# HK-SHAO/RayTracingPBR

Hardware: AMD Instinct MI355X
Metric: Msamples/sec (pixels x spp / s), Cornell Box 1920x1080 (higher is better)
Workload: dtype f32

## Files before the change

### raytracingpbr_amd/csrc/rt_capi.hip

```cpp
#include <hip/hip_runtime.h>

#include <cmath>
#include <cstdio>
#include <cstdlib>
#include <cstring>
#include <string>
#include <vector>

#include "rt_ctx.hpp"
#include "rt_features.hpp"
#include "rt_reproject.hpp"
#include "rt_noise.hpp"
#include "rt_present.hpp"
#include "rt_select.hpp"

using namespace rt;

static void derive_launch(rtpbr_ctx* c, RtJitKey* key, bool* want, bool* strict_error);
static int noise_alloc(rtpbr_ctx* c);
extern "C" int rtpbr_set_option(rtpbr_ctx* c, const char* key, long long value);
extern "C" int rtpbr_set_tiles(rtpbr_ctx* c, int tw, int th, int rank, int world);
extern "C" int rtpbr_set_camera(rtpbr_ctx* c, const rtpbr_camera* cam);

static thread_local char g_err[512];
// ... 648 lines not shown
        if (((mask >> b) & 1u) && c->read_pending[b] >= 0) {
            const hipError_t q = hipEventQuery(c->ev_read_done[c->read_pending[b] & 7]);
            if (q == hipErrorNotReady) {
                (void)hipGetLastError();
                HIP_TRY(hipStreamWaitEvent(c->stream, c->ev_read_done[c->read_pending[b] & 7], 0));
            } else if (q != hipSuccess) {
                return rt_fail_hip("hipEventQuery(read-back)", q);
            }
            c->read_pending[b] = -1;
        }
    return RTPBR_OK;
}
enum : unsigned { W_IMAGE_BUFFER = 1u << RTPBR_BUF_IMAGE_BUFFER, W_IMAGE_PIXELS = 1u << RTPBR_BUF_IMAGE_PIXELS, W_RAY_BUFFER = 1u << RTPBR_BUF_RAY_BUFFER,
                W_DIFF_BUFFER = 1u << RTPBR_BUF_DIFF_BUFFER, W_DIFF_PIXELS = 1u << RTPBR_BUF_DIFF_PIXELS };

extern "C" int rtpbr_refresh(rtpbr_ctx* c) {
    if (!c || !c->have_cfg) return fail(RTPBR_ESTATE, "set_config first");
    if (int r = set_dev(c)) return r;
    if (int r = flush_shade(c)) return r;
    if (int r = rt_order_after_reads(c, W_IMAGE_BUFFER | W_RAY_BUFFER | W_DIFF_BUFFER | W_DIFF_PIXELS | (c->noise_moments ? 1u << RTPBR_BUF_MOMENTS : 0u))) return r;
    size_t n = (size_t)c->cfg.width * c->cfg.height;
    if (c->noise_moments) {
        HIP_TRY(hipMemsetAsync(c->noise_moments, 0, n * sizeof(float4), c->stream));
        HIP_TRY(hipMemsetAsync(c->noise_snapshot, 0, n * sizeof(float4), c->stream));
    }
    launch_refresh(c->image_buffer, c->ray_buffer, c->diff_buffer, c->diff_pixels, c->cfg.adaptive_sampling, n, c->stream);
    HIP_TRY(hipGetLastError());
    c->history_ok = true;
    return RTPBR_OK;
}

static void pack_objects(rtpbr_ctx* c, Params& P) { pack_table(c->objm, c->n_obj, P.box_sig, P.objm); }

constexpr size_t PRIMARY_REC_BYTES = 5;
constexpr size_t STAGE_ITEM_BYTES = 14;
constexpr uint32_t DENSE_CHUNK_MIN = 32, DENSE_CHUNK_MAX = 256, DENSE_BATCH_MAX = 4096;
static size_t stage_bytes(size_t items) { return items * sizeof(StageRec) + (items / DENSE_CHUNK_MIN + 2) * sizeof(uint32_t) + items; }
static int staging_alloc(rtpbr_ctx* c, void** ptr, size_t* cap, size_t need) {
    if (need <= *cap) return RTPBR_OK;
    HIP_TRY(hipStreamSynchronize(c->stream));
    (void)hipFree(*ptr);
    *ptr = nullptr;
    *cap = 0;
    const hipError_t e = hipMalloc(ptr, need);
    if (e == hipErrorOutOfMemory) {
        (void)hipGetLastError();
        *ptr = nullptr;
        return RTPBR_ENOMEM;
    }
    if (e != hipSuccess) return rt_fail_hip("hipMalloc(staging)", e);
    *cap = need;
    return RTPBR_OK;
}
static int ensure_staging(rtpbr_ctx* c, size_t items, bool split, bool stage = true) {
    if (stage)
        if (int r = staging_alloc(c, (void**)&c->stage, &c->stage_cap, stage_bytes(items))) return r;
    if (split)
        if (int r = staging_alloc(c, (void**)&c->primary, &c->primary_cap, items * PRIMARY_REC_BYTES)) return r;
    return RTPBR_OK;
}

static int next_event_of(std::vector<hipEvent_t>& pool, int& used, hipEvent_t* out) {
    if (used == (int)pool.size()) {
        hipEvent_t e = nullptr;
        HIP_TRY(hipEventCreateWithFlags(&e, hipEventDisableSystemFence));
        pool.push_back(e);
    }
// ... 312 lines not shown
            c->shade_pending_base = P.sample_base;
            c->shade_pending_same_call = true;
        }
    }
    P.sparse_lanes = sparse_saved;
    return rc;
}

static int sample_complete_path(rtpbr_ctx* c, int n, bool selected = false) {
    Params& P = c->P;
    int left = n;
    if (int r = flush_shade(c)) return r;
    c->dense_launches = 0;
    const bool tracked = c->noise_tracking == RTPBR_NOISE_TRACK_SAMPLES;
    while (left > 0) {
        const bool split_ok = !selected && c->primary_split && P.scheduler == 1 && c->kind != KIND_BUNNY && c->kind != KIND_MIXED;
        const bool unstaged = c->precision != 0 && c->jit_mod != nullptr && P.scheduler == 1;
        long long per_spp = (long long)P.np * (long long)((unstaged ? 0 : STAGE_ITEM_BYTES) + (split_ok ? PRIMARY_REC_BYTES : 0));
        if (per_spp < 1) per_spp = 1;
        long long kmax = c->staging_bytes / per_spp;
        if (kmax < 1) kmax = 1;
        long long k32 = (0xFFFFFFFFLL - work_margin(c)) / (long long)P.np;
        if (k32 < 1) k32 = 1;
        if (kmax > k32) kmax = k32;
        int K = (int)(left < kmax ? left : kmax);
        const bool split = split_ok && (c->primary_split == 2 || (long long)P.np * K >= tune::PRIMARY_SPLIT_MIN_ITEMS);
        if (int r = ensure_staging(c, (size_t)P.np * (size_t)K, split, !unstaged)) {
            if (r != RTPBR_ENOMEM || K == 1)
                return r == RTPBR_ENOMEM ? fail(RTPBR_ENOMEM, "no device memory for the staging of one sample per pixel") : r;
            c->staging_bytes = (long long)((K + 1) / 2) * per_spp;
            continue;
        }
        P.primary = c->primary;
        P.primary_code = reinterpret_cast<uint8_t*>(c->primary + (size_t)P.np * (size_t)K);
        P.primary_split = split ? 1 : 0;
        P.primary_lean = c->primary_lean;
        P.drain_lanes = c->drain_lanes;
        P.stage = c->stage;
        P.K = K;
        P.sample_base = c->sample_base;
        P.total_items = (uint32_t)((long long)P.np * K);
        int grid = trace_grid(c, P.total_items, selected);
        long long waves = (long long)grid * tune::WAVES_PER_BLOCK;
        long long chunk = (long long)P.total_items / (waves * 64);
        if (chunk < tune::CHUNK_MIN) chunk = (long long)P.total_items < waves * tune::CHUNK_MIN ? tune::CHUNK_TINY : tune::CHUNK_MIN;
        if (chunk > tune::CHUNK_MAX) chunk = tune::CHUNK_MAX;
        if (c->chunk > 0) chunk = c->chunk;
        P.chunk = (uint32_t)chunk;
        P.stage_dense = 0;
        if (c->stage_dense && c->jit_mod != nullptr && !unstaged && P.scheduler == 1 && !tracked) {
            long long lo = DENSE_CHUNK_MIN, hi = chunk < 64 ? 64 : chunk > (long long)DENSE_CHUNK_MAX ? (long long)DENSE_CHUNK_MAX : chunk, cc = 0;
            if (c->chunk > 0) lo = hi = c->chunk;
            if (lo >= (long long)DENSE_CHUNK_MIN && hi <= (long long)DENSE_CHUNK_MAX)
                for (long long t = hi; t >= lo; t--)
                    if (t % K == 0 || K % t == 0) { cc = t; break; }
            const long long unit = cc > K ? cc : K;
            if (cc > 0 && unit <= (long long)DENSE_BATCH_MAX) {
                P.chunk = (uint32_t)cc;
                P.stage_dense = 1;
                c->dense_launches++;
                P.acc_batch = (uint32_t)(unit * ((long long)DENSE_BATCH_MAX / unit));
                P.acc_magic_k = K > 1 ? (uint32_t)(0x100000000ULL / (unsigned long long)K) + 1u : 0u;
                P.acc_magic_chunk = (uint32_t)(0x100000000ULL / (unsigned long long)cc) + 1u;
                const size_t n_fill = (size_t)P.total_items / (size_t)cc + 1;
                P.stage_fill = reinterpret_cast<uint32_t*>(c->stage + (size_t)P.total_items * 3u);
                P.stage_idx = reinterpret_cast<uint8_t*>(P.stage_fill + n_fill);
                HIP_TRY(hipMemsetAsync(P.stage_fill, 0, n_fill * sizeof(uint32_t), c->stream));
            }
// ... 1021 lines not shown
    } else if (!strcmp(key, "tiny_own")) {
        if (value < 0 || value > 128) return fail(RTPBR_EINVAL, "tiny_own must be 0 (no small heavy waves) .. 128");
        c->tiny_own = (int)value;
    } else if (!strcmp(key, "leave_x8")) {
        if (value < 1 || value > 4096) return fail(RTPBR_EINVAL, "leave_x8 must be 1 .. 4096 (eighths of a march iteration)");
        c->leave_x8 = (int)value;
    } else if (!strcmp(key, "heavy_prio")) {
        if (value < 0 || value > 1) return fail(RTPBR_EINVAL, "heavy_prio must be 0 or 1");
        c->heavy_prio = (int)value;
    } else if (!strcmp(key, "heavy_mean_x16")) {
        if (value < 0 || value > (1 << 20)) return fail(RTPBR_EINVAL, "heavy_mean_x16 must be 0 .. 2^20");
        c->heavy_mean_x16 = (int)value;
    } else if (!strcmp(key, "heavy_bulk_x16")) {
        if (value < 0 || value > (1 << 20)) return fail(RTPBR_EINVAL, "heavy_bulk_x16 must be 0 .. 2^20");
        c->heavy_bulk_x16 = (int)value;
    } else if (!strcmp(key, "grid_blocks")) {
        if (value < 0 || value > 65535) return fail(RTPBR_EINVAL, "grid_blocks must be 0 (automatic) .. 65535");
        c->grid_blocks = (int)value;
    } else if (!strcmp(key, "residency")) {
        if (value < 1 || value > 256 || (value & (value - 1))) return fail(RTPBR_EINVAL, "residency must be a power of two, 1..256");
        c->residency = (int)value;
    } else if (!strcmp(key, "ready_low")) {
        if (value < 0 || value > 63) return fail(RTPBR_EINVAL, "ready_low must be 0..63");
        c->ready_low = (int)value;
    } else if (!strcmp(key, "refill_lanes")) {
        if (value < 1 || value > 64) return fail(RTPBR_EINVAL, "refill_lanes must be 1..64");
        c->refill_lanes = (int)value;
    } else if (!strcmp(key, "timing")) {
        if (value < 0 || value > 1) return fail(RTPBR_EINVAL, "timing must be 0 or 1");
        c->timing = (int)value;
    } else if (!strcmp(key, "stage_dense")) {
        if (value < 0 || value > 1) return fail(RTPBR_EINVAL, "stage_dense must be 0 (item-linear staging) or 1 (records appended per claim in completion order)");
        c->stage_dense = (int)value;
    } else if (!strcmp(key, "primary_split")) {
        if (value < 0 || value > 2) return fail(RTPBR_EINVAL, "primary_split must be 0 (never), 1 (large launches) or 2 (always)");
        c->primary_split = (int)value;
    } else if (!strcmp(key, "drain_lanes")) {
        if (value < 0 || value > 64) return fail(RTPBR_EINVAL, "drain_lanes must be 0..64");
        c->drain_lanes = (int)value;
    } else if (!strcmp(key, "primary_lean")) {
        if (value < 0 || value > 1) return fail(RTPBR_EINVAL, "primary_lean must be 0 or 1");
        c->primary_lean = (int)value;
    } else if (!strcmp(key, "lazy_sqrt")) {
        if (value < 0 || value > 1) return fail(RTPBR_EINVAL, "lazy_sqrt must be 0 or 1");
        c->lazy_sqrt = (int)value;
    } else if (!strcmp(key, "jit")) {
        if (value < -1 || value > 2)
            return fail(RTPBR_EINVAL, "jit must be -1 (when no ahead-of-time specialisation fits), 0 (never), 1 (always, falling back to the "
                                      "ahead-of-time instance if compilation is impossible) or 2 (always, an error otherwise)");
        c->jit = (int)value;
    } else if (!strcmp(key, "precision")) {
        if (value < 0 || value > 1) return fail(RTPBR_EINVAL, "precision must be 0 (exactly rounded, the default) or 1 (tolerance flavour: hardware sqrt / rcp / sin / exp, contraction)");
        c->precision = (int)value;
    } else if (!strcmp(key, "jit_bake")) {
        if (value < 0 || value > 2) return fail(RTPBR_EINVAL, "jit_bake must be 0, 1 (scene + configuration) or 2 (+ the camera frame: fixed-camera offline renders)");
        c->jit_bake = (int)value;
    } else if (!strcmp(key, "specialize")) {
        if (value < 0 || value > 1) return fail(RTPBR_EINVAL, "specialize must be 0 or 1");
        c->specialize = (int)value;
    } else if (!strcmp(key, "mlp_mfma")) {
        if (value < 0 || value > 1) return fail(RTPBR_EINVAL, "mlp_mfma must be 0 or 1");
        c->mlp_mfma = (int)value;
    } else if (!strcmp(key, "mlp_lanes")) {
        if (value < 1 || value > 64) return fail(RTPBR_EINVAL, "mlp_lanes must be 1..64");
        c->mlp_lanes = (int)value;
    } else if (!strcmp(key, "mlp_full")) {
// ... 72 lines not shown
```

### raytracingpbr_amd/csrc/rt_ctx.hpp

```cpp
#pragma once
#include <hip/hip_runtime.h>

#include <string>
#include <vector>

#include "rt_device.hpp"
#include "rt_noise.hpp"
#include "rt_present.hpp"
#include "rt_select.hpp"

namespace rt {
void launch_trace(const Params& P, int kind, int grid, hipStream_t st);
void launch_accumulate(const Params& P, int n_cu, hipStream_t st);
void launch_trace_selected(const Params& P, int kind, int grid, hipStream_t st);
void launch_accumulate_selected(const Params& P, hipStream_t st);
void launch_accumulate_tracked(const Params& P, float4* moments, float4* snapshot, hipStream_t st);
void launch_accumulate_selected_tracked(const Params& P, float4* moments, float4* snapshot, hipStream_t st);
int trace_selected_blocks_per_cu(int kind, int n_obj, int scheduler);
void launch_zero(void* p, size_t bytes, hipStream_t st);
void launch_persistent(const Params& P, int kind, int steps, hipStream_t st);
void launch_persistent_pool(const Params& P, int kind, int steps, int grid, hipStream_t st);
int persistent_pool_blocks_per_cu(int kind);
void launch_chain_steps(const Params& P, int kind, int steps, int grid, hipStream_t st);
void launch_src_gen(const Params& P, int kind, hipStream_t st);
// ... 60 lines not shown
    using Params = rt::Params;
    using ObjFull = rt::ObjFull;
    using ObjM = rt::ObjM;
    using Counters = rt::Counters;
    static constexpr int MAX_OBJ = rt::MAX_OBJ;
    int device = 0;
    bool headless = false;
    hipStream_t stream = nullptr;
    bool have_cfg = false, have_scene = false, have_cam = false;
    rtpbr_config cfg{};
    rtpbr_object obj[MAX_OBJ];
    int n_obj = 0;
    int kind = rt::KIND_GENERIC;
    rtpbr_camera cam{};
    Params P{};
    float4* image_buffer = nullptr;
    float* image_pixels = nullptr;
    rtpbr_ray* ray_buffer = nullptr;
    float2* diff_buffer = nullptr;
    float* diff_pixels = nullptr;
    ObjFull* objfull = nullptr;
    float4* env = nullptr;
    uint32_t* env8 = nullptr;
    float* env_lut = nullptr;
    int env_packed = 1;
    float* bunny = nullptr;
    float* stage = nullptr;
    size_t stage_cap = 0;
    float* primary = nullptr;
    size_t primary_cap = 0;
    int drain_lanes = 16;
    int primary_lean = 1;
    int primary_split = 1;
    int specialize = 1;
    int lazy_sqrt = 1;
    uint32_t scene_sig = 0;
    ObjM objm[MAX_OBJ];
    unsigned int* work_counter = nullptr;
    int timing = 1;
    bool total1_recorded = false;
    Counters* counters = nullptr;
    Counters* counters_buf[2] = {nullptr, nullptr};
    bool counters_clean[2] = {false, false};
    int counters_turn = 0;
    int tile_w = 0, tile_h = 0, rank = 0, world = 1;
    uint32_t sample_base = 0;
    long long staging_bytes = 16LL << 30;
    int wait_lanes = 24;
    int shade_lanes = 56;
    int refill_lanes = 24;
    int ready_low = 4;
    int jit_waves = 0;
    int chunk = 0;
    int stage_dense = 0;
    unsigned long long dense_launches = 0;
    int residency = 32;
    int sparse_lanes = 24;
    int src_plan = 1;
    int plan_interval = 64;
    int heavy_own = 80;
    int age_on = 1;
    int age_w[8] = {8, 8, 8, 8, 8, 8, 8, 8};
    int tiny_waves = 64;
    int tiny_own = 8;
    int leave_x8 = 24;
    int src_track = 2;
    int src_op = 7;
    int heavy_prio = 1;
    int heavy_mean_x16 = 48;
    int heavy_bulk_x16 = 8;
    uint32_t* cost_buffer = nullptr;
    unsigned int* team_counter = nullptr;
    std::vector<void*> host_blocks;
    std::vector<size_t> host_sizes;
    hipStream_t copy_stream = nullptr;
    hipEvent_t ev_read_ready = nullptr;
    hipEvent_t ev_read_done[8] = {};
    int read_issued = 0;
    int read_pending[15] = {-1, -1, -1, -1, -1, -1, -1, -1, -1, -1, -1, -1, -1, -1, -1};
    uint32_t* march_out = nullptr;
// ... 84 lines not shown
```

### raytracingpbr_amd/csrc/rt_trace.hpp

```cpp
#pragma once
#include <hip/hip_runtime.h>

#include "rt_device.hpp"

namespace rt {

RT_D uint32_t wave_sum(uint32_t v) {
#pragma unroll
    for (int off = 32; off > 0; off >>= 1) v += __shfl_xor(v, off, 64);
    return v;
}

RT_D void flush_counters(const Params& P, uint32_t steps, uint32_t raycasts, uint32_t hits, uint32_t sky,
                         uint32_t samples, uint32_t deposits) {
    __shared__ unsigned long long blk[6];
    if (threadIdx.x < 6) blk[threadIdx.x] = 0;
    __syncthreads();
    steps = wave_sum(steps);
    raycasts = wave_sum(raycasts);
    hits = wave_sum(hits);
    sky = wave_sum(sky);
    samples = wave_sum(samples);
    deposits = wave_sum(deposits);
    if ((threadIdx.x & 63) == 0) {
// ... 140 lines not shown
}
RT_D void acc_flush_all(const Params& P, const AccView& A, int lane, uint32_t& n_dep) {
    lds_wave_fence();
    for (uint32_t s = 0; s < (uint32_t)ACC_SLOTS; s++) {
        const uint32_t t = (uint32_t)__builtin_amdgcn_readfirstlane((int)A.tag[s]);
        if (t != 0xffffffffu) acc_flush_slot(P, A, s, t, lane, n_dep);
    }
}

template <bool LIST = false>
RT_D int start_item(const Params& P, PathRay& R) {
    uint32_t q = R.item / (uint32_t)P.K;
    uint32_t k = R.item - q * (uint32_t)P.K;
    int px, py;
    if constexpr (LIST) {
        const uint32_t i = P.order[q];
        px = (int)(i / (uint32_t)P.cfg.height);
        py = (int)(i - (uint32_t)px * (uint32_t)P.cfg.height);
    } else {
        if (!pixel_of(P, q, px, py)) return -1;
    }
    R.key = rng_key(P.cfg.seed, (uint32_t)px, (uint32_t)py, P.sample_base + k);
    R.cnt = 0;
    gen_ray(P, px, py, R.key, R.cnt, R.o, R.d);
    R.col = mk(1, 1, 1);
    R.bounce = 0;
    float inv_pdf = exp_(0.0f / P.cfg.light_quality);
    float p = 1.0f - 1.0f / inv_pdf;
    if (rng_next(R.key, R.cnt) < p) {
        R.col = R.col * p;
        return 0;
    }
    return 1;
}

struct WorkRange {
    uint32_t next, end;
    bool drained;
};

RT_D bool claim_items(const Params& P, WorkRange& wr, bool want, int lane, uint32_t& item) {
    const unsigned long long m = __ballot(want);
    int need = __popcll(m);
    const int rank = (int)__builtin_amdgcn_mbcnt_hi((uint32_t)(m >> 32), __builtin_amdgcn_mbcnt_lo((uint32_t)m, 0));
    int assigned = 0;
    bool got = false;
    while (need > 0) {
        if (wr.next == wr.end) {
            if (wr.drained) break;
            uint32_t start = 0;
            if (lane == 0) start = atomicAdd(P.work_counter, P.chunk);
            start = __builtin_amdgcn_readfirstlane(start);
            if (start >= P.total_items) {
                wr.drained = true;
                break;
            }
            wr.next = start;
            uint32_t e = start + P.chunk;
            wr.end = e < P.total_items ? e : P.total_items;
        }
        int avail = (int)(wr.end - wr.next);
        int take = need < avail ? need : avail;
        if (want && !got && rank >= assigned && rank < assigned + take) {
            item = wr.next + (uint32_t)(rank - assigned);
            got = true;
        }
// ... 127 lines not shown
        const float t_before = L.t;
        int idx;
        float dist;
        uint32_t ev_mask = 0;
        uint32_t dbg_ev = 0;
        nearest_culled<KIND, NOBJ, SIG>(P, pos, L.t, active, ub, lb, idx, dist, dbg_hist ? &dbg_ev : nullptr, &ev_mask);
        if (dbg_hist) dbg_hist[dbg_ev < 8u ? dbg_ev : 8u]++;
        if (active) {
            L.t_eval = L.t;
            march_update(P, L, idx, dist);
        }
        const float moved = fabs_(L.t - t_before) * 1.000001f;
        ub = dist + moved;
#pragma unroll
        for (int i = 0; i < (NOBJ > 0 ? NOBJ : 1); i++) lb[i] -= moved;
        if (P.primary_lean && (ev_mask & (ev_mask - 1u)) == 0u && ev_mask != 0u) {
            const int k = (int)__builtin_ctz(ev_mask);
            uint32_t lean_iters = 0;
            static_for<(NOBJ > 0 ? NOBJ : 1), 1>([&](auto Ic) {
                constexpr int i = decltype(Ic)::value;
                if (k == i) primary_lean_obj<KIND, NOBJ, SIG, i>(P, L, ub, lb, lean_iters);
            });
            if (dbg_hist) dbg_hist[0] += lean_iters;
        }
    }
}

template <int KIND, int NOBJ, uint32_t SIG = 0, bool CULL = true>
RT_D void primary_rays_impl(const Params& P) {
    const int lane = threadIdx.x & 63;
    const uint32_t n_groups = (P.total_items + 63u) / 64u;
    const uint32_t n_waves = gridDim.x * 4u;
    uint32_t n_steps = 0, n_raycasts = 0;
#ifdef RT_DEBUG_PRIMARY
    uint32_t dbg_hist[9] = {0, 0, 0, 0, 0, 0, 0, 0, 0};
#endif
    uint32_t RUN = n_groups / (n_waves * 4u);
    RUN = RUN < 1u ? 1u : (RUN > 16u ? 16u : RUN);
    uint32_t g = 0, g_end = 0;
    for (;;) {
        if (g == g_end) {
            uint32_t start = 0;
            if (lane == 0) start = atomicAdd(P.work_counter + 1, RUN);
            g = __builtin_amdgcn_readfirstlane(start);
            if (g >= n_groups) break;
            g_end = g + RUN < n_groups ? g + RUN : n_groups;
        }
        const uint32_t item = g * 64u + (uint32_t)lane;
        g++;
        Lane L;
        L.state = ST_IDLE;
        L.n_steps = L.n_raycasts = L.n_hits = L.n_sky = 0;
        L.o = L.d = mk(0, 0, 0);
        L.t = L.w = L.s = L.dist = L.t_eval = 0.0f;
        L.idx = 0;
        L.steps_left = 0;
        PathRay R;
        R.item = item;
        bool valid = false;
        if (item < P.total_items) {
            int r = start_item(P, R);
            valid = r == 1;
            if (valid) {
                L.o = R.o;
                L.d = R.d;
                march_init(P, L);
            }
        }
        if constexpr (CULL && NOBJ > 0 && KIND != KIND_BUNNY && KIND != KIND_MIXED) {
#ifdef RT_DEBUG_PRIMARY
            culled_march_wave<KIND, NOBJ, SIG>(P, L, dbg_hist);
#else
            culled_march_wave<KIND, NOBJ, SIG>(P, L, nullptr);
#endif
        } else {
            while (__any(L.state == ST_MARCH)) {
                if (L.state == ST_MARCH) march_step<KIND, NOBJ, SIG>(P, L);
            }
        }
        if (item < P.total_items) {
            P.primary[item] = L.t_eval;
            P.primary_code[item] = (uint8_t)((uint32_t)L.idx | ((uint32_t)(valid ? L.state : ST_IDLE) << 5));
        }
        n_steps += L.n_steps;
        n_raycasts += L.n_raycasts;
    }
#ifdef RT_DEBUG_PRIMARY
    if (lane == 0)
        for (int i = 0; i < 9; i++) atomicAdd(&P.counters->dbg[i], (unsigned long long)dbg_hist[i]);
#endif
    flush_counters(P, n_steps, n_raycasts, 0, 0, 0, 0);
}

template <int KIND, int NOBJ, uint32_t SIG = 0>
__global__ void __launch_bounds__(256) primary_rays(const Params P) { primary_rays_impl<KIND, NOBJ, SIG>(P); }

enum { SL_EMPTY = 0, SL_READY = 1, SL_HIT = 2, SL_MISS = 3 };
constexpr int POOL_WORDS = 15;

struct PoolView {
    uint32_t (*pool)[64];
    uint32_t* sstate;
    uint32_t* tbl;
};

RT_D void lds_wave_fence() {
#if defined(__HIP_DEVICE_COMPILE__)
    __builtin_amdgcn_fence(__ATOMIC_RELEASE, "wavefront");
    __builtin_amdgcn_wave_barrier();
    __builtin_amdgcn_fence(__ATOMIC_ACQUIRE, "wavefront");
#endif
}
RT_D int wave_rank(unsigned long long m) {
    return (int)__builtin_amdgcn_mbcnt_hi((uint32_t)(m >> 32), __builtin_amdgcn_mbcnt_lo((uint32_t)m, 0));
}
template <int W>
RT_D void pool_load(const PoolView& V, uint32_t slot, uint32_t (&rec)[W]) {
#pragma unroll
    for (int w = 0; w < W; w++) rec[w] = V.pool[w][slot];
}
template <int W>
RT_D void pool_store(const PoolView& V, uint32_t slot, const uint32_t (&rec)[W]) {
#pragma unroll
    for (int w = 0; w < W; w++) V.pool[w][slot] = rec[w];
// ... 111 lines not shown
    const int m_swap = P.swap_lanes;

    auto f2u = [](float x) { return __builtin_bit_cast(uint32_t, x); };
    auto u2f = [](uint32_t x) { return __builtin_bit_cast(float, x); };

#ifdef RT_DEBUG_CULL
    float dbg_lb[NOBJ > 0 ? NOBJ : 1];
#pragma unroll
    for (int i = 0; i < (NOBJ > 0 ? NOBJ : 1); i++) dbg_lb[i] = -1.0f;
    float dbg_ub = 3.0e38f;
    uint32_t dbg_cull_eval = 0, dbg_cull_all = 0;
#endif
#ifdef RT_DEBUG_PHASE
    unsigned long long tB = 0, tD = 0, tA = 0, tc = __builtin_readcyclecounter();
    unsigned long long dbg_march_lanes = 0, dbg_march_steps = 0, dbg_shade_lanes = 0, dbg_shade_passes = 0;
#define RT_PHASE(acc) { unsigned long long tn = __builtin_readcyclecounter(); acc += tn - tc; tc = tn; }
#else
#define RT_PHASE(acc)
#endif
    for (;;) {
        {
            const int n_shade = __popcll(m_shade);
            const int n_ready = __popcll(m_ready);
            const int n_free = 64 - n_shade - n_ready;
            const bool run_b = n_shade >= T || (n_ready <= P.ready_low && (n_shade > 0 || (n_free > 0 && !wr.drained)));
            if (run_b) {
                if constexpr (KIND == KIND_BOXES || KIND == KIND_GENERIC) {
                    float (*sv)[64] = save_all[wave];
                    sv[0][lane] = L.o.x, sv[1][lane] = L.o.y, sv[2][lane] = L.o.z;
                    sv[3][lane] = L.d.x, sv[4][lane] = L.d.y, sv[5][lane] = L.d.z;
                    sv[6][lane] = L.dist;
                }
                uint32_t st = sstate[lane];
                w_hits += (uint32_t)__popcll(__ballot(st == SL_HIT));
                PathRay R;
                R.o = R.d = R.col = mk(0, 0, 0);
                R.t_eval = 0.0f;
                R.idx = R.bounce = 0;
                R.key = R.cnt = R.item = 0;
                bool alive = false;
                uint32_t sky1 = 0;
                if (st == SL_HIT || st == SL_MISS) {
                    R.o = mk(u2f(pool[F_OX][lane]), u2f(pool[F_OY][lane]), u2f(pool[F_OZ][lane]));
                    R.d = mk(u2f(pool[F_DX][lane]), u2f(pool[F_DY][lane]), u2f(pool[F_DZ][lane]));
                    R.col = mk(u2f(pool[F_CR][lane]), u2f(pool[F_CG][lane]), u2f(pool[F_CB][lane]));
                    R.t_eval = u2f(pool[F_TEVAL][lane]);
                    const uint32_t meta = pool[F_META][lane];
                    R.idx = meta_idx(meta);
                    R.bounce = meta_bounce(meta);
                    R.cnt = meta_cnt(meta);
                    R.key = pool[F_KEY][lane];
                    R.item = pool[F_ITEM][lane];
                    if (KIND != KIND_BUNNY) {
                        if (st == SL_HIT) {
                            alive = shade_hit<KIND>(P, lds_obj, R);
                        } else {
                            shade_miss(P, R, sky1);
                        }
                    }
                }
                if (KIND == KIND_BUNNY) {
                    vec3 hp = fma3(R.t_eval, R.d, R.o);
                    vec3 nrm = mk(0, 0, 0);
                    if (__any(st == SL_HIT)) {
                        w_mlp_lane += 4u * (uint32_t)__popcll(__ballot(st == SL_HIT));
                        if (P.mlp_mfma) nrm = bunny_normal_wave(P, b_frag, b_lds, b_bias, tbl_w, lane, st == SL_HIT, hp, w_mlp_wave);
                        else if (st == SL_HIT) nrm = calc_normal<KIND_BUNNY>(P, lds_obj[0], hp);
                    }
                    if (st == SL_HIT) {
                        alive = shade_hit<KIND, true>(P, lds_obj, R, nrm);
                    } else if (st == SL_MISS) {
                        shade_miss(P, R, sky1);
                    }
                }
                w_sky += (uint32_t)__popcll(__ballot(sky1 != 0));
#if RT_FAST_MATH
                acc_add(P, A, (st == SL_HIT || st == SL_MISS) && !alive, R.item / (uint32_t)P.K, R.col, lane, n_dep);
#else
                stage_sample(P, (st == SL_HIT || st == SL_MISS) && !alive, R.item, R.col, lane);
#endif
                w_samples += (uint32_t)__popcll(__ballot((st == SL_HIT || st == SL_MISS) && !alive));
                if (st == SL_HIT || st == SL_MISS) st = SL_EMPTY;
                const bool is_free = st == SL_EMPTY && !alive;
                const bool do_refill = __popcll(__ballot(is_free)) >= P.refill_lanes || n_shade < T;
                bool got = claim_items(P, wr, is_free && do_refill, lane, R.item);
                uint32_t resumed = 0;
                bool roulette0 = false;
                float rec_t = 0.0f;
                uint32_t rec_code = 0;
                if (got && P.primary_split) {
#if defined(__HIP_DEVICE_COMPILE__)
                    rec_t = __builtin_nontemporal_load(P.primary + R.item);
                    rec_code = __builtin_nontemporal_load(P.primary_code + R.item);
#else
                    rec_t = P.primary[R.item];
                    rec_code = P.primary_code[R.item];
#endif
                }
                if (got) {
                    int r = start_item<LIST>(P, R);
                    if (r == 1) {
                        if (P.primary_split) {
                            R.t_eval = rec_t;
                            R.idx = (int)(rec_code & 31u);
                            resumed = rec_code >> 5;
                        } else {
                            alive = true;
                        }
                    }
                    roulette0 = r == 0;
                }
#if RT_FAST_MATH
                acc_add(P, A, roulette0, R.item / (uint32_t)P.K, R.col, lane, n_dep);
#else
#if RT_STAGE_DENSE
                if (__any(roulette0)) stage_sample(P, roulette0, R.item, R.col, lane);
#else
                if (roulette0) write_sample(P, R.item, R.col);
#endif
#endif
                w_samples += (uint32_t)__popcll(__ballot(roulette0));
                if (resumed == ST_HIT || resumed == ST_MISS) {
                    pool[F_OX][lane] = f2u(R.o.x); pool[F_OY][lane] = f2u(R.o.y); pool[F_OZ][lane] = f2u(R.o.z);
                    pool[F_DX][lane] = f2u(R.d.x); pool[F_DY][lane] = f2u(R.d.y); pool[F_DZ][lane] = f2u(R.d.z);
                    pool[F_CR][lane] = f2u(R.col.x); pool[F_CG][lane] = f2u(R.col.y); pool[F_CB][lane] = f2u(R.col.z);
                    pool[F_TEVAL][lane] = f2u(R.t_eval);
                    pool[F_META][lane] = pack_meta(R.idx, R.bounce, R.cnt);
                    pool[F_KEY][lane] = R.key;
                    pool[F_ITEM][lane] = R.item;
                    st = resumed == ST_HIT ? SL_HIT : SL_MISS;
                }
                if (alive) {
                    pool[F_OX][lane] = f2u(R.o.x); pool[F_OY][lane] = f2u(R.o.y); pool[F_OZ][lane] = f2u(R.o.z);
                    pool[F_DX][lane] = f2u(R.d.x); pool[F_DY][lane] = f2u(R.d.y); pool[F_DZ][lane] = f2u(R.d.z);
                    pool[F_CR][lane] = f2u(R.col.x); pool[F_CG][lane] = f2u(R.col.y); pool[F_CB][lane] = f2u(R.col.z);
                    pool[F_META][lane] = pack_meta(0, R.bounce, R.cnt);
                    pool[F_KEY][lane] = R.key;
                    pool[F_ITEM][lane] = R.item;
                    st = SL_READY;
                }
                sstate[lane] = st;
                m_ready = __ballot(st == SL_READY);
                m_shade = __ballot(st == SL_HIT || st == SL_MISS);
                if constexpr (KIND == KIND_BOXES || KIND == KIND_GENERIC) {
                    float (*sv)[64] = save_all[wave];
                    L.o = mk(sv[0][lane], sv[1][lane], sv[2][lane]);
                    L.d = mk(sv[3][lane], sv[4][lane], sv[5][lane]);
                    L.dist = sv[6][lane];
                }
            }
        }

        RT_PHASE(tB)
        {
            const bool is_done = L.state == ST_HIT || L.state == ST_MISS;
            uint32_t rec[F_COUNT];
            rec[F_OX] = f2u(L.o.x); rec[F_OY] = f2u(L.o.y); rec[F_OZ] = f2u(L.o.z);
            rec[F_DX] = f2u(L.d.x); rec[F_DY] = f2u(L.d.y); rec[F_DZ] = f2u(L.d.z);
            rec[F_CR] = f2u(a_col.x); rec[F_CG] = f2u(a_col.y); rec[F_CB] = f2u(a_col.z);
            rec[F_TEVAL] = f2u(L.t_eval);
            rec[F_META] = (a_meta & ~31u) | (uint32_t)L.idx;
            rec[F_KEY] = a_key; rec[F_ITEM] = a_item;
            const int r = pool_swap(V, lane, is_done, L.state == ST_IDLE, L.state == ST_HIT ? SL_HIT : SL_MISS, rec, m_ready, m_shade);
            if (r & 2) L.state = ST_IDLE;
            w_raycasts += (uint32_t)__popcll(__ballot((r & 1) != 0));
            if (r & 1) {
                L.o = mk(u2f(rec[F_OX]), u2f(rec[F_OY]), u2f(rec[F_OZ]));
                L.d = mk(u2f(rec[F_DX]), u2f(rec[F_DY]), u2f(rec[F_DZ]));
                a_col = mk(u2f(rec[F_CR]), u2f(rec[F_CG]), u2f(rec[F_CB]));
                a_meta = rec[F_META];
                a_key = rec[F_KEY]; a_item = rec[F_ITEM];
                march_init(P, L);
// ... 138 lines not shown
```

### raytracingpbr_amd/csrc/rt_types.hpp

```cpp
#pragma once
#include <stdint.h>

#include "../../include/rtpbr.h"
#include "rt_math.hpp"

namespace rt {

constexpr int MAX_OBJ = RTPBR_MAX_OBJECTS;
static_assert(sizeof(rtpbr_config) == 164 && sizeof(rtpbr_object) == 116 && sizeof(rtpbr_camera) == 52 &&
                  sizeof(rtpbr_ray) == 40,
              "C-ABI struct layout changed");

enum { ROT_GENERAL = 0, ROT_IDENT = 1, ROT_X = 2, ROT_Y = 3, ROT_Z = 4 };
#define RT_BOX_SIGNATURES(X, ...) X(0x4db691u, __VA_ARGS__)

constexpr int sig_cls(uint32_t sig, int i) { return (int)((sig >> (3 * i)) & 7u); }
constexpr int sig_words(int cls) { return cls == ROT_GENERAL ? 16 : (cls == ROT_IDENT ? 8 : 12); }
constexpr int sig_offset(uint32_t sig, int i) {
    int o = 0;
    for (int j = 0; j < i; j++) o += sig_words(sig_cls(sig, j));
    return o;
}

#ifndef RT_JIT_TYPES
// ... 36 lines not shown
struct CamFrame {
    float lf[3], x[3], y[3], llc[3], hor[3], ver[3];
    float lens_radius;
    float inv_w, inv_h;
};
static_assert(sizeof(CamFrame) == 21 * 4, "RtJitKey::cam_words holds a CamFrame");

struct __attribute__((packed, aligned(4))) StageRec { float r, g, b; };
static_assert(sizeof(StageRec) == 12, "staging record is 12 bytes");

struct Counters {
    unsigned long long samples, raycasts, march_steps, hits, sky_lookups, deposits;
    unsigned long long mlp_wave_evals, mlp_lane_evals;
    unsigned long long dbg[32];
    unsigned long long shard[64][16];
};

struct PlanBuf {
    uint32_t hist[256];
    uint32_t cursor[256];
    unsigned long long total;
    uint32_t n_heavy;
    uint32_t tiny_waves;
    uint32_t n_chain, n_chain_waves;
    uint32_t chain_start[2049];
    uint32_t age_valid;
    uint32_t age_cls;
    uint32_t age_w[8];
    float age_wf[8];
    unsigned long long life_sum[8];
    uint32_t life_cnt[8];
};

struct Params {
    rtpbr_config cfg;
    CamFrame cam;
    int32_t n_obj;
    float anim_s, anim_c;
    float anim_bz;
    uint32_t sample_base;
    int32_t K;
    int32_t tile_w, tile_h, ntx, nty, rank, world;
    int32_t n_local_tiles;
    int32_t np;
    uint32_t total_items;
    uint32_t chunk;
    int32_t wait_lanes;
    int32_t shade_lanes;
    int32_t refill_lanes;
    int32_t ready_low;
    int32_t swap_lanes;
    int32_t sparse_lanes;
    int32_t heavy_own;
    int32_t n_cu;
    int32_t age_on;
    uint32_t age_pack;
    int32_t tiny_own;
    int32_t leave_x8;
    int32_t chain_on;
    int32_t src_track;
    int32_t src_op;
    int32_t split_head;
    int32_t heavy_prio;
    int32_t scheduler;
    int32_t mlp_mfma;
    int32_t mlp_lanes;
// ... 46 lines not shown
```

Before: 4405.

## Store full primary ray records and retire constant-color primary misses early

The primary-split pass now saves the full primary ray (t, key, direction, origin for non-pinhole cameras) in a column layout. The wavefront refill path can then resume an item from that record instead of calling start_item again to rebuild the camera ray. Primary misses with a black or white miss color are written directly in the primary pass and skipped later, and an optional refill-before-shade ordering is added. The default staging budget is doubled to fit the larger per-item records, which raises memory traffic and footprint.

```diff
diff --git a/raytracingpbr_amd/csrc/rt_capi.hip b/raytracingpbr_amd/csrc/rt_capi.hip
--- a/raytracingpbr_amd/csrc/rt_capi.hip
+++ b/raytracingpbr_amd/csrc/rt_capi.hip
@@ -704,7 +704,7 @@
 
 static void pack_objects(rtpbr_ctx* c, Params& P) { pack_table(c->objm, c->n_obj, P.box_sig, P.objm); }
 
-constexpr size_t PRIMARY_REC_BYTES = 5;
+constexpr size_t PRIMARY_REC_BYTES = 4 * PRIMARY_REC_COLS + 1;
 constexpr size_t STAGE_ITEM_BYTES = 14;
 constexpr uint32_t DENSE_CHUNK_MIN = 32, DENSE_CHUNK_MAX = 256, DENSE_BATCH_MAX = 4096;
 static size_t stage_bytes(size_t items) { return items * sizeof(StageRec) + (items / DENSE_CHUNK_MIN + 2) * sizeof(uint32_t) + items; }
@@ -1083,8 +1083,9 @@
             continue;
         }
         P.primary = c->primary;
-        P.primary_code = reinterpret_cast<uint8_t*>(c->primary + (size_t)P.np * (size_t)K);
-        P.primary_split = split ? 1 : 0;
+        P.primary_code = reinterpret_cast<uint8_t*>(c->primary + (size_t)PRIMARY_REC_COLS * (size_t)P.np * (size_t)K);
+        const bool retire = split && c->primary_retire && !unstaged && !(c->stage_dense && c->jit_mod != nullptr && !tracked);
+        P.primary_split = split ? PS_SPLIT | (c->refill_first ? PS_REFILL_FIRST : 0) | (retire ? PS_RETIRE : 0) : 0;
         P.primary_lean = c->primary_lean;
         P.drain_lanes = c->drain_lanes;
         P.stage = c->stage;
@@ -2172,6 +2173,12 @@
     } else if (!strcmp(key, "stage_dense")) {
         if (value < 0 || value > 1) return fail(RTPBR_EINVAL, "stage_dense must be 0 (item-linear staging) or 1 (records appended per claim in completion order)");
         c->stage_dense = (int)value;
+    } else if (!strcmp(key, "refill_first")) {
+        if (value < 0 || value > 1) return fail(RTPBR_EINVAL, "refill_first must be 0 or 1");
+        c->refill_first = (int)value;
+    } else if (!strcmp(key, "primary_retire")) {
+        if (value < 0 || value > 1) return fail(RTPBR_EINVAL, "primary_retire must be 0 or 1");
+        c->primary_retire = (int)value;
     } else if (!strcmp(key, "primary_split")) {
         if (value < 0 || value > 2) return fail(RTPBR_EINVAL, "primary_split must be 0 (never), 1 (large launches) or 2 (always)");
         c->primary_split = (int)value;
diff --git a/raytracingpbr_amd/csrc/rt_ctx.hpp b/raytracingpbr_amd/csrc/rt_ctx.hpp
--- a/raytracingpbr_amd/csrc/rt_ctx.hpp
+++ b/raytracingpbr_amd/csrc/rt_ctx.hpp
@@ -116,6 +116,8 @@
     int drain_lanes = 16;
     int primary_lean = 1;
     int primary_split = 1;
+    int refill_first = 0;
+    int primary_retire = 1;
     int specialize = 1;
     int lazy_sqrt = 1;
     uint32_t scene_sig = 0;
@@ -129,7 +131,7 @@
     int counters_turn = 0;
     int tile_w = 0, tile_h = 0, rank = 0, world = 1;
     uint32_t sample_base = 0;
-    long long staging_bytes = 16LL << 30;
+    long long staging_bytes = 32LL << 30;
     int wait_lanes = 24;
     int shade_lanes = 56;
     int refill_lanes = 24;
diff --git a/raytracingpbr_amd/csrc/rt_trace.hpp b/raytracingpbr_amd/csrc/rt_trace.hpp
--- a/raytracingpbr_amd/csrc/rt_trace.hpp
+++ b/raytracingpbr_amd/csrc/rt_trace.hpp
@@ -196,6 +196,36 @@
         return 0;
     }
     return 1;
+}
+
+RT_D uint32_t primary_draws(const Params& P) { return P.cfg.camera_kind == RTPBR_CAMERA_PINHOLE ? 3u : 5u; }
+template <class T>
+RT_D T load_once(const T* p) {
+#if defined(__HIP_DEVICE_COMPILE__)
+    return __builtin_nontemporal_load(p);
+#else
+    return *p;
+#endif
+}
+RT_D uint32_t resume_item(const Params& P, PathRay& R) {
+    const size_t n = P.total_items;
+    const float* const c = P.primary + R.item;
+    const uint32_t code = load_once(P.primary_code + R.item);
+    R.t_eval = load_once(c + PC_TEVAL * n);
+    R.key = __builtin_bit_cast(uint32_t, load_once(c + PC_KEY * n));
+    R.d = mk(load_once(c + PC_DX * n), load_once(c + PC_DY * n), load_once(c + PC_DZ * n));
+    if (P.cfg.camera_kind == RTPBR_CAMERA_PINHOLE) R.o = mk(P.cam.lf[0], P.cam.lf[1], P.cam.lf[2]);
+    else R.o = mk(load_once(c + PC_OX * n), load_once(c + PC_OY * n), load_once(c + PC_OZ * n));
+    R.col = mk(1, 1, 1);
+    R.bounce = 0;
+    R.cnt = primary_draws(P);
+    R.idx = (int)(code & 31u);
+    return code >> 5;
+}
+RT_D vec3 roulette0_color(const Params& P) {
+    const float inv_pdf = exp_(0.0f / P.cfg.light_quality);
+    const float p = 1.0f - 1.0f / inv_pdf;
+    return mk(1, 1, 1) * p;
 }
 
 struct WorkRange {
@@ -389,6 +419,9 @@
     const uint32_t n_groups = (P.total_items + 63u) / 64u;
     const uint32_t n_waves = gridDim.x * 4u;
     uint32_t n_steps = 0, n_raycasts = 0;
+    uint32_t w_samples = 0;
+    const bool miss_black = P.cfg.sky_kind == RTPBR_SKY_BLACK || P.cfg.primary_miss == RTPBR_PRIMARY_BLACK;
+    const bool retire = (P.primary_split & PS_RETIRE) != 0 && (miss_black || P.cfg.primary_miss == RTPBR_PRIMARY_WHITE);
 #ifdef RT_DEBUG_PRIMARY
     uint32_t dbg_hist[9] = {0, 0, 0, 0, 0, 0, 0, 0, 0};
 #endif
@@ -414,10 +447,11 @@
         L.steps_left = 0;
         PathRay R;
         R.item = item;
-        bool valid = false;
+        bool valid = false, roulette0 = false;
         if (item < P.total_items) {
             int r = start_item(P, R);
             valid = r == 1;
+            roulette0 = r == 0;
             if (valid) {
                 L.o = R.o;
                 L.d = R.d;
@@ -435,10 +469,24 @@
                 if (L.state == ST_MARCH) march_step<KIND, NOBJ, SIG>(P, L);
             }
         }
+        bool retired = false;
         if (item < P.total_items) {
-            P.primary[item] = L.t_eval;
-            P.primary_code[item] = (uint8_t)((uint32_t)L.idx | ((uint32_t)(valid ? L.state : ST_IDLE) << 5));
-        }
+            uint32_t rec = valid ? (L.state == ST_HIT ? REC_HIT : REC_MISS) : roulette0 ? REC_ROULETTE : REC_NONE;
+            if (retire && rec == REC_MISS) {
+                write_sample(P, item, miss_black ? mk(0, 0, 0) : mk(1, 1, 1));
+                rec = REC_RETIRED;
+            } else if (valid) {
+                const size_t n = P.total_items;
+                float* const c = P.primary + item;
+                c[PC_TEVAL * n] = L.t_eval;
+                c[PC_KEY * n] = __builtin_bit_cast(float, R.key);
+                c[PC_DX * n] = L.d.x, c[PC_DY * n] = L.d.y, c[PC_DZ * n] = L.d.z;
+                if (P.cfg.camera_kind != RTPBR_CAMERA_PINHOLE) c[PC_OX * n] = L.o.x, c[PC_OY * n] = L.o.y, c[PC_OZ * n] = L.o.z;
+            }
+            P.primary_code[item] = (uint8_t)((uint32_t)L.idx | (rec << 5));
+            retired = rec == REC_RETIRED;
+        }
+        w_samples += (uint32_t)__popcll(__ballot(retired));
         n_steps += L.n_steps;
         n_raycasts += L.n_raycasts;
     }
@@ -446,7 +494,7 @@
     if (lane == 0)
         for (int i = 0; i < 9; i++) atomicAdd(&P.counters->dbg[i], (unsigned long long)dbg_hist[i]);
 #endif
-    flush_counters(P, n_steps, n_raycasts, 0, 0, 0, 0);
+    flush_counters(P, n_steps, n_raycasts, 0, 0, lane == 0 ? w_samples : 0u, 0);
 }
 
 template <int KIND, int NOBJ, uint32_t SIG = 0>
@@ -624,112 +672,142 @@
                     sv[6][lane] = L.dist;
                 }
                 uint32_t st = sstate[lane];
-                w_hits += (uint32_t)__popcll(__ballot(st == SL_HIT));
                 PathRay R;
                 R.o = R.d = R.col = mk(0, 0, 0);
                 R.t_eval = 0.0f;
                 R.idx = R.bounce = 0;
                 R.key = R.cnt = R.item = 0;
-                bool alive = false;
-                uint32_t sky1 = 0;
-                if (st == SL_HIT || st == SL_MISS) {
-                    R.o = mk(u2f(pool[F_OX][lane]), u2f(pool[F_OY][lane]), u2f(pool[F_OZ][lane]));
-                    R.d = mk(u2f(pool[F_DX][lane]), u2f(pool[F_DY][lane]), u2f(pool[F_DZ][lane]));
-                    R.col = mk(u2f(pool[F_CR][lane]), u2f(pool[F_CG][lane]), u2f(pool[F_CB][lane]));
-                    R.t_eval = u2f(pool[F_TEVAL][lane]);
-                    const uint32_t meta = pool[F_META][lane];
-                    R.idx = meta_idx(meta);
-                    R.bounce = meta_bounce(meta);
-                    R.cnt = meta_cnt(meta);
-                    R.key = pool[F_KEY][lane];
-                    R.item = pool[F_ITEM][lane];
-                    if (KIND != KIND_BUNNY) {
-                        if (st == SL_HIT) {
-                            alive = shade_hit<KIND>(P, lds_obj, R);
+                const bool split = (P.primary_split & PS_SPLIT) != 0;
+                const bool refill_first = (P.primary_split & PS_REFILL_FIRST) != 0;
+                bool fresh = false;
+#pragma nounroll
+                for (int step = 0; step < 2; step++) {
+                    if ((step == 0) != refill_first) {
+                        w_hits += (uint32_t)__popcll(__ballot(st == SL_HIT));
+                        const bool waits = st == SL_HIT || st == SL_MISS;
+                        bool alive = false;
+                        uint32_t sky1 = 0;
+                        if (waits) {
+                            if (!fresh) {
+                                R.o = mk(u2f(pool[F_OX][lane]), u2f(pool[F_OY][lane]), u2f(pool[F_OZ][lane]));
+                                R.d = mk(u2f(pool[F_DX][lane]), u2f(pool[F_DY][lane]), u2f(pool[F_DZ][lane]));
+                                R.col = mk(u2f(pool[F_CR][lane]), u2f(pool[F_CG][lane]), u2f(pool[F_CB][lane]));
+                                R.t_eval = u2f(pool[F_TEVAL][lane]);
+                                const uint32_t meta = pool[F_META][lane];
+                                R.idx = meta_idx(meta);
+                                R.bounce = meta_bounce(meta);
+                                R.cnt = meta_cnt(meta);
+                                R.key = pool[F_KEY][lane];
+                                R.item = pool[F_ITEM][lane];
+                            }
+                            if (KIND != KIND_BUNNY) {
+                                if (st == SL_HIT) {
+                                    alive = shade_hit<KIND>(P, lds_obj, R);
+                                } else {
+                                    shade_miss(P, R, sky1);
+                                }
+                            }
+                        }
+                        if (KIND == KIND_BUNNY) {
+                            vec3 hp = fma3(R.t_eval, R.d, R.o);
+                            vec3 nrm = mk(0, 0, 0);
+                            if (__any(st == SL_HIT)) {
+                                w_mlp_lane += 4u * (uint32_t)__popcll(__ballot(st == SL_HIT));
+                                if (P.mlp_mfma) nrm = bunny_normal_wave(P, b_frag, b_lds, b_bias, tbl_w, lane, st == SL_HIT, hp, w_mlp_wave);
+                                else if (st == SL_HIT) nrm = calc_normal<KIND_BUNNY>(P, lds_obj[0], hp);
+                            }
+                            if (st == SL_HIT) {
+                                alive = shade_hit<KIND, true>(P, lds_obj, R, nrm);
+                            } else if (st == SL_MISS) {
+                                shade_miss(P, R, sky1);
+                            }
+                        }
+                        w_sky += (uint32_t)__popcll(__ballot(sky1 != 0));
+#if RT_FAST_MATH
+                        acc_add(P, A, waits && !alive, R.item / (uint32_t)P.K, R.col, lane, n_dep);
+#else
+                        stage_sample(P, waits && !alive, R.item, R.col, lane);
+#endif
+                        w_samples += (uint32_t)__popcll(__ballot(waits && !alive));
+                        if (alive) {
+                            pool[F_OX][lane] = f2u(R.o.x); pool[F_OY][lane] = f2u(R.o.y); pool[F_OZ][lane] = f2u(R.o.z);
+                            pool[F_DX][lane] = f2u(R.d.x); pool[F_DY][lane] = f2u(R.d.y); pool[F_DZ][lane] = f2u(R.d.z);
+                            pool[F_CR][lane] = f2u(R.col.x); pool[F_CG][lane] = f2u(R.col.y); pool[F_CB][lane] = f2u(R.col.z);
+                            pool[F_META][lane] = pack_meta(0, R.bounce, R.cnt);
+                            pool[F_KEY][lane] = R.key;
+                            pool[F_ITEM][lane] = R.item;
+                            st = SL_READY;
+                        } else if (waits) {
+                            st = SL_EMPTY;
+                        }
+                    } else {
+                        bool want = st == SL_EMPTY;
+                        want = want && (__popcll(__ballot(want)) >= P.refill_lanes || n_shade < T);
+                        if (split) {
+                            constexpr int RECLAIM_MAX = 16;
+                            for (int round = 0;; round++) {
+                                uint32_t item = 0;
+                                const bool got = claim_items(P, wr, want, lane, item);
+                                uint32_t rec = REC_NONE;
+                                if (got) {
+                                    R.item = item;
+                                    rec = resume_item(P, R);
+                                }
+                                if (__any(rec == REC_ROULETTE)) {
+                                    const bool r0 = rec == REC_ROULETTE;
+                                    const vec3 c0 = roulette0_color(P);
+#if RT_FAST_MATH
+                                    acc_add(P, A, r0, item / (uint32_t)P.K, c0, lane, n_dep);
+#else
+                                    stage_sample(P, r0, item, c0, lane);
+#endif
+                                    w_samples += (uint32_t)__popcll(__ballot(r0));
+                                }
+                                if (rec == REC_HIT || rec == REC_MISS) {
+                                    st = rec == REC_HIT ? SL_HIT : SL_MISS;
+                                    if (refill_first) {
+                                        fresh = true;
+                                    } else {
+                                        pool[F_OX][lane] = f2u(R.o.x); pool[F_OY][lane] = f2u(R.o.y); pool[F_OZ][lane] = f2u(R.o.z);
+                                        pool[F_DX][lane] = f2u(R.d.x); pool[F_DY][lane] = f2u(R.d.y); pool[F_DZ][lane] = f2u(R.d.z);
+                                        pool[F_CR][lane] = f2u(R.col.x); pool[F_CG][lane] = f2u(R.col.y); pool[F_CB][lane] = f2u(R.col.z);
+                                        pool[F_TEVAL][lane] = f2u(R.t_eval);
+                                        pool[F_META][lane] = pack_meta(R.idx, R.bounce, R.cnt);
+                                        pool[F_KEY][lane] = R.key;
+                                        pool[F_ITEM][lane] = R.item;
+                                    }
+                                }
+                                want = got && st == SL_EMPTY;
+                                if (round + 1 == RECLAIM_MAX || __popcll(__ballot(want)) < P.refill_lanes) break;
+                            }
                         } else {
-                            shade_miss(P, R, sky1);
+                            const bool got = claim_items(P, wr, want, lane, R.item);
+                            bool roulette0 = false;
+                            if (got) {
+                                const int r = start_item<LIST>(P, R);
+                                roulette0 = r == 0;
+                                if (r == 1) {
+                                    pool[F_OX][lane] = f2u(R.o.x); pool[F_OY][lane] = f2u(R.o.y); pool[F_OZ][lane] = f2u(R.o.z);
+                                    pool[F_DX][lane] = f2u(R.d.x); pool[F_DY][lane] = f2u(R.d.y); pool[F_DZ][lane] = f2u(R.d.z);
+                                    pool[F_CR][lane] = f2u(R.col.x); pool[F_CG][lane] = f2u(R.col.y); pool[F_CB][lane] = f2u(R.col.z);
+                                    pool[F_META][lane] = pack_meta(0, R.bounce, R.cnt);
+                                    pool[F_KEY][lane] = R.key;
+                                    pool[F_ITEM][lane] = R.item;
+                                    st = SL_READY;
+                                }
+                            }
+#if RT_FAST_MATH
+                            acc_add(P, A, roulette0, R.item / (uint32_t)P.K, R.col, lane, n_dep);
+#else
+#if RT_STAGE_DENSE
+                            if (__any(roulette0)) stage_sample(P, roulette0, R.item, R.col, lane);
+#else
+                            if (roulette0) write_sample(P, R.item, R.col);
+#endif
+#endif
+                            w_samples += (uint32_t)__popcll(__ballot(roulette0));
                         }
                     }
-                }
-                if (KIND == KIND_BUNNY) {
-                    vec3 hp = fma3(R.t_eval, R.d, R.o);
-                    vec3 nrm = mk(0, 0, 0);
-                    if (__any(st == SL_HIT)) {
-                        w_mlp_lane += 4u * (uint32_t)__popcll(__ballot(st == SL_HIT));
-                        if (P.mlp_mfma) nrm = bunny_normal_wave(P, b_frag, b_lds, b_bias, tbl_w, lane, st == SL_HIT, hp, w_mlp_wave);
-                        else if (st == SL_HIT) nrm = calc_normal<KIND_BUNNY>(P, lds_obj[0], hp);
-                    }
-                    if (st == SL_HIT) {
-                        alive = shade_hit<KIND, true>(P, lds_obj, R, nrm);
-                    } else if (st == SL_MISS) {
-                        shade_miss(P, R, sky1);
-                    }
-                }
-                w_sky += (uint32_t)__popcll(__ballot(sky1 != 0));
-#if RT_FAST_MATH
-                acc_add(P, A, (st == SL_HIT || st == SL_MISS) && !alive, R.item / (uint32_t)P.K, R.col, lane, n_dep);
-#else
-                stage_sample(P, (st == SL_HIT || st == SL_MISS) && !alive, R.item, R.col, lane);
-#endif
-                w_samples += (uint32_t)__popcll(__ballot((st == SL_HIT || st == SL_MISS) && !alive));
-                if (st == SL_HIT || st == SL_MISS) st = SL_EMPTY;
-                const bool is_free = st == SL_EMPTY && !alive;
-                const bool do_refill = __popcll(__ballot(is_free)) >= P.refill_lanes || n_shade < T;
-                bool got = claim_items(P, wr, is_free && do_refill, lane, R.item);
-                uint32_t resumed = 0;
-                bool roulette0 = false;
-                float rec_t = 0.0f;
-                uint32_t rec_code = 0;
-                if (got && P.primary_split) {
-#if defined(__HIP_DEVICE_COMPILE__)
-                    rec_t = __builtin_nontemporal_load(P.primary + R.item);
-                    rec_code = __builtin_nontemporal_load(P.primary_code + R.item);
-#else
-                    rec_t = P.primary[R.item];
-                    rec_code = P.primary_code[R.item];
-#endif
-                }
-                if (got) {
-                    int r = start_item<LIST>(P, R);
-                    if (r == 1) {
-                        if (P.primary_split) {
-                            R.t_eval = rec_t;
-                            R.idx = (int)(rec_code & 31u);
-                            resumed = rec_code >> 5;
-                        } else {
-                            alive = true;
-                        }
-                    }
-                    roulette0 = r == 0;
-                }
-#if RT_FAST_MATH
-                acc_add(P, A, roulette0, R.item / (uint32_t)P.K, R.col, lane, n_dep);
-#else
-#if RT_STAGE_DENSE
-                if (__any(roulette0)) stage_sample(P, roulette0, R.item, R.col, lane);
-#else
-                if (roulette0) write_sample(P, R.item, R.col);
-#endif
-#endif
-                w_samples += (uint32_t)__popcll(__ballot(roulette0));
-                if (resumed == ST_HIT || resumed == ST_MISS) {
-                    pool[F_OX][lane] = f2u(R.o.x); pool[F_OY][lane] = f2u(R.o.y); pool[F_OZ][lane] = f2u(R.o.z);
-                    pool[F_DX][lane] = f2u(R.d.x); pool[F_DY][lane] = f2u(R.d.y); pool[F_DZ][lane] = f2u(R.d.z);
-                    pool[F_CR][lane] = f2u(R.col.x); pool[F_CG][lane] = f2u(R.col.y); pool[F_CB][lane] = f2u(R.col.z);
-                    pool[F_TEVAL][lane] = f2u(R.t_eval);
-                    pool[F_META][lane] = pack_meta(R.idx, R.bounce, R.cnt);
-                    pool[F_KEY][lane] = R.key;
-                    pool[F_ITEM][lane] = R.item;
-                    st = resumed == ST_HIT ? SL_HIT : SL_MISS;
-                }
-                if (alive) {
-                    pool[F_OX][lane] = f2u(R.o.x); pool[F_OY][lane] = f2u(R.o.y); pool[F_OZ][lane] = f2u(R.o.z);
-                    pool[F_DX][lane] = f2u(R.d.x); pool[F_DY][lane] = f2u(R.d.y); pool[F_DZ][lane] = f2u(R.d.z);
-                    pool[F_CR][lane] = f2u(R.col.x); pool[F_CG][lane] = f2u(R.col.y); pool[F_CB][lane] = f2u(R.col.z);
-                    pool[F_META][lane] = pack_meta(0, R.bounce, R.cnt);
-                    pool[F_KEY][lane] = R.key;
-                    pool[F_ITEM][lane] = R.item;
-                    st = SL_READY;
                 }
                 sstate[lane] = st;
                 m_ready = __ballot(st == SL_READY);
diff --git a/raytracingpbr_amd/csrc/rt_types.hpp b/raytracingpbr_amd/csrc/rt_types.hpp
--- a/raytracingpbr_amd/csrc/rt_types.hpp
+++ b/raytracingpbr_amd/csrc/rt_types.hpp
@@ -92,6 +92,12 @@
     uint32_t life_cnt[8];
 };
 
+enum { PC_TEVAL = 0, PC_KEY, PC_DX, PC_DY, PC_DZ, PC_OX, PC_OY, PC_OZ, PRIMARY_REC_COLS };
+enum { REC_NONE = 0, REC_ROULETTE = 1, REC_HIT = 2, REC_MISS = 3, REC_RETIRED = 4 };
+enum { PS_SPLIT = 1,
+       PS_REFILL_FIRST = 2,
+       PS_RETIRE = 4 };
+
 struct Params {
     rtpbr_config cfg;
     CamFrame cam;
```

New measurement: 4391. Within noise of the previous version (-0.3%).
